# IannLiu/ReactRanker

Measured on AMD Instinct MI355X. Metric: queries/sec (lists scored+loss) ListMLE, higher is better.
Workload: dtype f32; 1 GPU; ListMLE 100k queries x 64 candidates (BASELINE.json configs[2]), 64-query steps, D-MPNN depth=3 hidden=300; preset=mle64, phase=train step: fwd + loss + bwd + grad all-reduce + Adam/NoamLR, candidates_per_query=64, pad_width_K=4, step_pool=6, parallelism=dp1

## Files before the change

### reactranker_amd/csrc/linear_common.h

```cpp
#pragma once
#include "rr_common.h"

namespace {

constexpr int BM = 64;
constexpr int BK = 16;
constexpr int THREADS = 256;

enum : int {
  F_A1_VEC = 1, F_A2_VEC = 2, F_SUB_VEC = 4, F_MASK_VEC = 8, F_W1_VEC = 16, F_W2_VEC = 32, F_EPI_VEC = 64, F_PRE_VEC = 128
};

__host__ __device__ constexpr int r16(int k) { return (k + 15) & ~15; }

struct LinearParams {
  rr_linear_args a;
  int w_k1_off;
  int t1, t2;
  int flags;
  uint32_t drop_thr;
  float keep_scale;
  int persist;
};

__device__ __forceinline__ f32x4 ld4(const float* p) { return *reinterpret_cast<const f32x4*>(p); }
typedef const __attribute__((address_space(1))) f32x4* rr_gptr4;
typedef const __attribute__((address_space(1))) int32_t* rr_gptri;
__device__ __forceinline__ f32x4 ldg4(const float* p) { return *(rr_gptr4)(p); }
__device__ __forceinline__ int32_t ldgi(const int32_t* p) { return *(rr_gptri)(p); }
typedef const __attribute__((address_space(1))) uint8_t* rr_gptrb;
__device__ __forceinline__ uint32_t ldgb(const uint8_t* p) { return *(rr_gptrb)(p); }
__host__ __device__ constexpr int64_t mask_bits_row(int N) { return 40 * ((N + 303) / 304); }

__device__ __forceinline__ void rr_glds16(const float* gsrc, uint32_t lds_dst) {
  uint32_t keep;
  asm volatile("s_mov_b32 %0, m0\n\ts_mov_b32 m0, %2\n\ts_nop 0\n\tglobal_load_lds_dwordx4 %1, off\n\ts_mov_b32 m0, %0"
               : "=&s"(keep)
               : "v"(gsrc), "s"(lds_dst)
               : "memory");
}
__device__ __forceinline__ void rr_wait_vm0() { asm volatile("s_waitcnt vmcnt(0)" ::: "memory"); }
__device__ __forceinline__ uint32_t rr_lds_addr(const float* p) {
  return static_cast<uint32_t>(reinterpret_cast<uintptr_t>((const __attribute__((address_space(3))) float*)p));
}

__device__ __forceinline__ f32x4 load_chunk(const float* p, int k, int ks, bool vec) {
  f32x4 v = f32x4(0.f);
  if (p == nullptr || k >= ks) return v;
  if (vec) {
    v = ld4(p + k);
    if (k + 3 >= ks) {
      if (k + 1 >= ks) v.y = 0.f;
      if (k + 2 >= ks) v.z = 0.f;
      v.w = 0.f;
    }
  } else {
    v.x = p[k];
    if (k + 1 < ks) v.y = p[k + 1];
    if (k + 2 < ks) v.z = p[k + 2];
    if (k + 3 < ks) v.w = p[k + 3];
  }
  return v;
}

__device__ __forceinline__ f32x4 apply_mask(f32x4 v, f32x4 mk, float scale) {
  v.x = mk.x > 0.f ? v.x * scale : 0.f;
  v.y = mk.y > 0.f ? v.y * scale : 0.f;
  v.z = mk.z > 0.f ? v.z * scale : 0.f;
  v.w = mk.w > 0.f ? v.w * scale : 0.f;
  return v;
}

#ifdef RR_TRACE
__device__ unsigned long long* rr_trace_buf = nullptr;
#define RR_STAMP(slot)                                                                                   \
  do {                                                                                                   \
    if (rr_trace_buf && threadIdx.x == 0 && blockIdx.y == 0) {                                           \
      rr_trace_buf[static_cast<size_t>(blockIdx.x) * 8 + (slot)] = __builtin_amdgcn_s_memrealtime();     \
      if ((slot) == 1) rr_trace_buf[static_cast<size_t>(blockIdx.x) * 8 + 5] = __builtin_amdgcn_s_memtime(); \
      if ((slot) == 2) rr_trace_buf[static_cast<size_t>(blockIdx.x) * 8 + 6] = __builtin_amdgcn_s_memtime(); \
    }                                                                                                    \
  } while (0)
inline int rr_trace_set_unit(unsigned long long* buf) {
  return hipMemcpyToSymbol(HIP_SYMBOL(rr_trace_buf), &buf, sizeof(buf)) == hipSuccess ? 0 : 1;
}
#else
#define RR_STAMP(slot)
#endif

__device__ __attribute__((aligned(16))) const float rr_zero_chunk[4] = {0.f, 0.f, 0.f, 0.f};
constexpr int RR_ZERO_ROW = 1024;
__device__ __attribute__((aligned(16))) const float rr_zero_row[RR_ZERO_ROW] = {0.f};

typedef __bf16 bf16x8 __attribute__((ext_vector_type(8)));
typedef uint32_t u32x4 __attribute__((ext_vector_type(4)));

constexpr int SK = 32;

__host__ __device__ constexpr int r32(int k) { return (k + 31) & ~31; }

__device__ __forceinline__ uint32_t cvt_pk_bf16(float lo, float hi) {
  uint32_t r;
  asm("v_cvt_pk_bf16_f32 %0, %1, %2" : "=v"(r) : "v"(lo), "v"(hi));
  return r;
}
__device__ __forceinline__ void split_pair(float x, float y, uint32_t& p0, uint32_t& p1, uint32_t& p2) {
  p0 = cvt_pk_bf16(x, y);
  float rx = x - __uint_as_float(p0 << 16), ry = y - __uint_as_float(p0 & 0xffff0000u);
  p1 = cvt_pk_bf16(rx, ry);
  rx -= __uint_as_float(p1 << 16);
  ry -= __uint_as_float(p1 & 0xffff0000u);
  p2 = cvt_pk_bf16(rx, ry);
}
__device__ __forceinline__ bf16x8 as_bf16x8(u32x4 v) { return __builtin_bit_cast(bf16x8, v); }
typedef _Float16 f16x8 __attribute__((ext_vector_type(8)));
typedef _Float16 f16x2 __attribute__((ext_vector_type(2)));
typedef float f32x2 __attribute__((ext_vector_type(2)));
__device__ __forceinline__ f16x8 as_f16x8(u32x4 v) { return __builtin_bit_cast(f16x8, v); }
__host__ __device__ __forceinline__ int rr_f16_exp(float bound) {
  uint32_t u;
  __builtin_memcpy(&u, &bound, 4);
  int e = static_cast<int>((u >> 23) & 0xffu) - 127;
  return e < -110 ? -110 : (e > 110 ? 110 : e);
}
__device__ __forceinline__ float rr_amax4(float m, f32x4 v) {
  return fmaxf(fmaxf(m, fmaxf(fabsf(v.x), fabsf(v.y))), fmaxf(fabsf(v.z), fabsf(v.w)));
}
__device__ __forceinline__ void rr_amax_commit_wave(float m, unsigned int* lds_word) {
#pragma unroll
  for (int o = 32; o > 0; o >>= 1) m = fmaxf(m, __shfl_xor(m, o));
  if ((threadIdx.x & 63) == 0 && m > 0.f) atomicMax(lds_word, __float_as_uint(m));
}
__device__ __forceinline__ float rr_pow2(int e) { return __uint_as_float(static_cast<uint32_t>(127 + e) << 23); }
__device__ __forceinline__ void split_pair_h(float x, float y, float S, uint32_t& p0, uint32_t& p1) {
  const f32x2 v = {x * S, y * S};
  const f16x2 h = __builtin_convertvector(v, f16x2);
  p0 = __builtin_bit_cast(uint32_t, h);
  const f32x2 r = v - __builtin_convertvector(h, f32x2);
  p1 = __builtin_bit_cast(uint32_t, __builtin_convertvector(r, f16x2));
}

inline bool vec_ok(const float* p, int64_t ld) { return p && rr_aligned16(p) && (ld % 4 == 0); }

inline LinearParams linear_params(const rr_linear_args& a) {
  LinearParams P;
  P.a = a;
  P.w_k1_off = a.w_packed ? r16(a.k1) : a.k1;
  P.t1 = (a.k1 + BK - 1) / BK;
  P.t2 = (a.k2 + BK - 1) / BK;
  P.flags = 0;
  P.persist = 0;
  if (a.k1 > 0 && vec_ok(a.a1, a.lda1)) P.flags |= F_A1_VEC;
  if (a.k2 > 0 && vec_ok(a.a2, a.lda2)) P.flags |= F_A2_VEC;
  if (a.a1_sub && vec_ok(a.a1_sub, a.lda1_sub)) P.flags |= F_SUB_VEC;
  if (a.a_mask && vec_ok(a.a_mask, a.ld_mask)) P.flags |= F_MASK_VEC;
  if (vec_ok(a.w, a.ldw)) {
    P.flags |= F_W1_VEC;
    if (a.k1 % 4 == 0) P.flags |= F_W2_VEC;
  }
  if (a.w_packed) P.flags |= F_W1_VEC | F_W2_VEC;
  if (a.N % 4 == 0 && vec_ok(a.c, a.ldc) && (!a.bias || rr_aligned16(a.bias)) &&
      (!a.residual || vec_ok(a.residual, a.ldr)))
    P.flags |= F_EPI_VEC;
  if (a.c_pre && vec_ok(a.c_pre, a.ld_pre)) P.flags |= F_PRE_VEC;
  P.drop_thr = rr_drop_threshold(a.drop_p);
  P.keep_scale = 1.0f / (1.0f - a.drop_p);
  return P;
}
}

extern "C" __attribute__((visibility("hidden"))) int rr_linear_split_launch(const rr_linear_args* args, int two_f16, rr_stream_t stream);
#ifdef RR_TRACE
extern "C" __attribute__((visibility("hidden"))) int rr_trace_set_linear_split(unsigned long long* buf);
extern "C" __attribute__((visibility("hidden"))) int rr_trace_set_wgrad(unsigned long long* buf);
#endif
```

### reactranker_amd/csrc/linear_split.hip

```cpp
#include "linear_common.h"
#include <atomic>

namespace {

#ifndef RR_EPI_MODE
#define RR_EPI_MODE 1
#endif

__host__ __device__ constexpr bool split_lean(int k1, int k2) { return k1 + SK <= RR_ZERO_ROW && k2 + SK <= RR_ZERO_ROW; }
__host__ __device__ constexpr bool split_can_persist(int NTP, int NT, int MODE, int WAVES, int EPI) {
  return MODE == 0 && WAVES == 12 && NT == NTP && EPI == 0;
}

template <int NTP, int NT, int MODE, int WAVES, int EPI = 0, bool F16 = false>
__global__ void __launch_bounds__(64 * WAVES, WAVES == 8 ? 4 : 3) linear_split_kernel(const LinearParams P) {
  constexpr int BN = 16 * NT;
  constexpr int TERMS = F16 ? 2 : 3;
  constexpr int PANEL = NT * TERMS * 1024;
  constexpr int SRC_PANEL = NTP * TERMS * 1024;
  constexpr int S_THREADS = 64 * WAVES;
  extern __shared__ __attribute__((aligned(16))) unsigned char smem[];
  constexpr bool RS_EPI = WAVES == 12;
  constexpr int RS = 77, REGION = 8 * RS * 16;
  constexpr int CS_OFF = RS_EPI ? (WAVES * REGION > 2 * PANEL ? WAVES * REGION : 2 * PANEL) : 0;
  constexpr int BIAS_OFF = RS_EPI ? CS_OFF + WAVES * BN * 4 : 2 * PANEL;
  float* const bias_s = reinterpret_cast<float*>(smem + BIAS_OFF);
  constexpr int PF_OFF = BIAS_OFF + BN * 4;
  constexpr bool PAIR = NTP == 2 * NT;
  const unsigned int bx = PAIR ? (((blockIdx.x >> 4) << 3) + (blockIdx.x & 7u)) : blockIdx.x;
  const unsigned int by = PAIR ? ((blockIdx.x >> 3) & 1u) : blockIdx.y;
  if (PAIR && static_cast<int64_t>(bx) * (16 * WAVES) >= P.a.M) return;
  const int t0 = by * NT;
  const int nth = NTP - t0 < NT ? NTP - t0 : NT;
  const bool full = nth == NT;
  const int n0 = t0 * 16;

  const rr_linear_args& a = P.a;
  const int tid = threadIdx.x, lane = tid & 63, wave = tid >> 6;
  const int fr = lane & 15, fkq = lane >> 4;
  float xs = 1.f, ixs = 1.f, iws = 1.f;
  if (F16) {
    float b1 = (a.a1_amax ? rr_amax_read(a.a1_amax) : 0.f) + (a.a1_sub_amax ? rr_amax_read(a.a1_sub_amax) : 0.f);
    if (MODE == 2 || MODE == 3) b1 *= fabsf(a.mask_scale);
    const float b2 = a.a2_amax ? rr_amax_read(a.a2_amax) : 0.f;
    const float bound = fmaxf(b1, b2);
    const int e = rr_f16_exp(bound);
    xs = bound < 2.5e33f ? rr_pow2(14 - e) : __builtin_nanf("");
    ixs = rr_pow2(e - 14);
    iws = 1.0f / a.w[static_cast<int64_t>(P.t1 + P.t2) * (SRC_PANEL / 4)];
  }
  RR_STAMP(0);
#ifdef RR_TRACE
  if (rr_trace_buf && threadIdx.x == 0 && by == 0) {
    unsigned hw, xcc;
    asm volatile("s_getreg_b32 %0, hwreg(HW_REG_HW_ID)" : "=s"(hw));
    asm volatile("s_getreg_b32 %0, hwreg(HW_REG_XCC_ID)" : "=s"(xcc));
    rr_trace_buf[static_cast<size_t>(bx) * 8 + 4] = (static_cast<unsigned long long>(xcc) << 32) | hw;
  }
#endif
#ifdef RR_SPLIT_STAGGER
  if (WAVES == 12 && gridDim.x > 256 && blockIdx.x < 256) {
    const int ph = (blockIdx.x >> 3) & 3;
    for (int i = 0; i < ph * RR_SPLIT_STAGGER; ++i) __builtin_amdgcn_s_sleep(127);
  }
#endif
  constexpr bool CAN_PERSIST = split_can_persist(NTP, NT, MODE, WAVES, EPI);
  const bool persist = CAN_PERSIST && P.persist != 0;
  unsigned int* const amx = reinterpret_cast<unsigned int*>(smem + PF_OFF + (CAN_PERSIST ? WAVES * 2048 : 0));
  if (F16 && tid == 0) { amx[0] = 0u; amx[1] = 0u; }
  int64_t g_cur = static_cast<int64_t>(bx) * WAVES;
  int64_t g_end = g_cur + WAVES;
  if (persist) {
    const int64_t units = (a.M + 63) / 64, G = gridDim.x;
    const int64_t base = units / G, rem = units % G, p = blockIdx.x;
    g_cur = 4 * (p * base + (p < rem ? p : rem));
    g_end = g_cur + 4 * (base + (p < rem ? 1 : 0));
  }
  int nw = g_end - g_cur < WAVES ? static_cast<int>(g_end - g_cur) : WAVES;
  int64_t m0 = g_cur * 16;
  int64_t m = m0 + wave * 16 + fr;
  bool row_ok = wave < nw && m < a.M;
  int64_t mc = row_ok ? m : a.M - 1;
  const float* const dummy = a.w;
  const float* rowp1 = nullptr;
  const float* rowp2 = nullptr;
  const float* subp = nullptr;
  const uint8_t* bitrow = nullptr;
  {
    const bool g1 = a.k1 > 0 && a.a1_idx != nullptr;
    const bool g2 = MODE == 1 && a.k1 > 0 && a.a1_sub != nullptr && a.a1_sub_idx != nullptr;
    const int32_t j1 = g1 ? ldgi(a.a1_idx + mc) : 0;
    const int32_t j2 = g2 ? ldgi(a.a1_sub_idx + mc) : 0;
    if (row_ok) {
      if (a.k1 > 0) {
        if (g1) {
          if (j1 >= 0) rowp1 = a.a1 + static_cast<int64_t>(j1) * a.lda1;
        } else {
          rowp1 = a.a1 + m * a.lda1;
        }
        if (MODE == 1 && a.a1_sub) {
          if (g2) {
            if (j2 >= 0) subp = a.a1_sub + static_cast<int64_t>(j2) * a.lda1_sub;
          } else {
            subp = a.a1_sub + m * a.lda1_sub;
          }
        }
        if (MODE == 2) subp = a.a_mask + m * a.ld_mask;
        if (MODE == 3) bitrow = a.a_mask_bits + m * mask_bits_row(a.k1);
      }
      if (a.k2 > 0) rowp2 = a.a2 + m * a.lda2;
    }
  }
  float dz_am = 0.f;
  float* dzrow = nullptr;
  if ((MODE == 2 || MODE == 3) && a.dz_out && row_ok && by == 0) dzrow = a.dz_out + m * a.ld_dz;

  const int uwave = __builtin_amdgcn_readfirstlane(wave);
  const float* const wlane = a.w + t0 * (TERMS * 256) + lane * 4;
  const uint32_t lds0 = rr_lds_addr(reinterpret_cast<const float*>(smem));

  f32x4 acc[NT];
#pragma unroll
  for (int i = 0; i < NT; ++i) acc[i] = f32x4(0.f);

  const int nk = P.t1 + P.t2;
  f32x4 ra[WAVES == 12 ? 2 : 1][2], rs[WAVES == 12 ? 2 : 1][2];
  uint32_t rb[2] = {0u, 0u};
  u32x4 x0, x1, x2;

#ifndef RR_SPLIT_NO_FASTX
  constexpr bool FASTX = (MODE == 0 || MODE == 1);
#else
  constexpr bool FASTX = false;
#endif
  static_assert(RR_ZERO_ROW % SK == 0 && RR_ZERO_ROW >= 2 * SK, "rr_zero_row must hold whole k-steps");
  constexpr bool LEAN_ONLY = FASTX && WAVES == 12 && EPI < 2;
  const bool fastx_ok = FASTX && (LEAN_ONLY || split_lean(a.k1, a.k2));
  const float* xb1 = (rowp1 != nullptr ? rowp1 : rr_zero_row) + fkq * 8;
  const float* xb2 = (rowp2 != nullptr ? rowp2 : rr_zero_row) + fkq * 8;
  const float* const sb1 = (subp != nullptr ? subp : rr_zero_row) + fkq * 8;
  const float* xb1n = xb1;
  const float* xb2n = xb2;
  bool has_next = false, wrapped = false;
  auto next_rows = [&](int64_t g, int nwn) {
    const int64_t mm = (g + wave) * 16 + fr;
    const bool ok = wave < nwn && mm < a.M;
    const int64_t mmc = ok ? mm : a.M - 1;
    const bool g1 = a.k1 > 0 && a.a1_idx != nullptr;
    const int32_t j1 = g1 ? ldgi(a.a1_idx + mmc) : 0;
    const float* r1 = nullptr;
    const float* r2 = nullptr;
    if (ok) {
      if (a.k1 > 0) {
        if (g1) {
          if (j1 >= 0) r1 = a.a1 + static_cast<int64_t>(j1) * a.lda1;
        } else {
          r1 = a.a1 + mm * a.lda1;
        }
      }
      if (a.k2 > 0) r2 = a.a2 + mm * a.lda2;
    }
    xb1n = (r1 != nullptr ? r1 : rr_zero_row) + fkq * 8;
    xb2n = (r2 != nullptr ? r2 : rr_zero_row) + fkq * 8;
  };
  auto interior = [&](int s) -> bool {
    if (!fastx_ok) return false;
    return s < P.t1 ? (s + 1) * SK <= a.k1 : (s - P.t1 + 1) * SK <= a.k2;
  };
  auto issue_x = [&](int s, int slot, bool nextblk = false) {
    if (FASTX && fastx_ok) {
      const bool s1 = s < P.t1;
      const int off = (s1 ? s : s - P.t1) * SK;
      const float* p = (s1 ? (nextblk ? xb1n : xb1) : (nextblk ? xb2n : xb2)) + off;
      const float* q = (MODE == 1 && s1) ? sb1 + off : rr_zero_row;
      if (interior(s)) {
        ra[slot][0] = ldg4(p);
        ra[slot][1] = ldg4(p + 4);
        if (MODE == 1) {
          rs[slot][0] = ldg4(q);
          rs[slot][1] = ldg4(q + 4);
        }
      } else {
        int fq = fkq;
        if (CAN_PERSIST) asm volatile("" : "+v"(fq));
        const int kl = off + fq * 8, ks = s1 ? a.k1 : a.k2;
        ra[slot][0] = ldg4(kl < ks ? p : rr_zero_row);
        ra[slot][1] = ldg4(kl + 4 < ks ? p + 4 : rr_zero_row);
        if (MODE == 1) {
          rs[slot][0] = ldg4(kl < ks ? q : rr_zero_row);
          rs[slot][1] = ldg4(kl + 4 < ks ? q + 4 : rr_zero_row);
        }
      }
      return;
    }
    const bool seg1 = s < P.t1;
    const int kl = (seg1 ? s : s - P.t1) * SK + fkq * 8;
    const float* p = seg1 ? rowp1 : rowp2;
    const int ks = seg1 ? a.k1 : a.k2;
    ra[slot][0] = ldg4((p != nullptr && kl < ks) ? p + kl : dummy);
    ra[slot][1] = ldg4((p != nullptr && kl + 4 < ks) ? p + kl + 4 : dummy);
    if (MODE == 1 || MODE == 2) {
      const bool oks = seg1 && subp != nullptr;
      rs[slot][0] = ldg4((oks && kl < ks) ? subp + kl : dummy);
      rs[slot][1] = ldg4((oks && kl + 4 < ks) ? subp + kl + 4 : dummy);
    }
    if (MODE == 3) {
      const int tc = 2 * s + (fkq >> 1);
      const int y = tc / 19;
      const uint8_t* q = bitrow + y * 40 + (fkq & 1) * 20 + (tc - 19 * y);
      rb[slot] = ldgb((seg1 && bitrow != nullptr && kl < ks) ? q : reinterpret_cast<const uint8_t*>(dummy));
    }
  };
  auto issue_w = [&](int s) {
    const float* src = wlane + static_cast<int64_t>(s) * (SRC_PANEL / 4);
    const uint32_t dst = lds0 + (s & 1) * PANEL;
#pragma unroll
    for (int b0 = 0; b0 < NT * TERMS; b0 += WAVES) {
      const int b = b0 + uwave;
      if (b < nth * TERMS) rr_glds16(src + b * 256, dst + b * 1024);
    }
  };
  auto split8 = [&](const f32x4& v0, const f32x4& v1) {
    uint32_t t0, t1, t2;
    if (F16) {
      split_pair_h(v0.x, v0.y, xs, t0, t1); x0.x = t0; x1.x = t1;
      split_pair_h(v0.z, v0.w, xs, t0, t1); x0.y = t0; x1.y = t1;
      split_pair_h(v1.x, v1.y, xs, t0, t1); x0.z = t0; x1.z = t1;
      split_pair_h(v1.z, v1.w, xs, t0, t1); x0.w = t0; x1.w = t1;
      return;
    }
    split_pair(v0.x, v0.y, t0, t1, t2); x0.x = t0; x1.x = t1; x2.x = t2;
    split_pair(v0.z, v0.w, t0, t1, t2); x0.y = t0; x1.y = t1; x2.y = t2;
    split_pair(v1.x, v1.y, t0, t1, t2); x0.z = t0; x1.z = t1; x2.z = t2;
    split_pair(v1.z, v1.w, t0, t1, t2); x0.w = t0; x1.w = t1; x2.w = t2;
  };
  auto fixup = [&](int s, int slot) {
    if (CAN_PERSIST && uwave >= nw) return;
    if (FASTX && fastx_ok) {
      f32x4 v0 = ra[slot][0], v1 = ra[slot][1];
      f32x4 u0 = f32x4(0.f), u1 = f32x4(0.f);
      if (MODE == 1) { u0 = rs[slot][0]; u1 = rs[slot][1]; }
      const bool s1 = s < P.t1;
      const int ks = s1 ? a.k1 : a.k2;
      if (!interior(s) && (ks & 3) != 0) {
        const int kl = (s1 ? s : s - P.t1) * SK + fkq * 8;
#pragma unroll
        for (int e = 0; e < 4; ++e) {
          v0[e] = kl + e < ks ? v0[e] : 0.f;
          v1[e] = kl + 4 + e < ks ? v1[e] : 0.f;
          if (MODE == 1) {
            u0[e] = kl + e < ks ? u0[e] : 0.f;
            u1[e] = kl + 4 + e < ks ? u1[e] : 0.f;
          }
        }
      }
      if (MODE == 1) {
        v0 = v0 - u0;
        v1 = v1 - u1;
      }
      split8(v0, v1);
      return;
    }
    const bool seg1 = s < P.t1;
    const int kl = (seg1 ? s : s - P.t1) * SK + fkq * 8;
    const float* p = seg1 ? rowp1 : rowp2;
    const int ks = seg1 ? a.k1 : a.k2;
    const bool ok = (p != nullptr);
    f32x4 v0, v1;
#pragma unroll
    for (int e = 0; e < 4; ++e) {
      v0[e] = (ok && kl + e < ks) ? ra[slot][0][e] : 0.f;
      v1[e] = (ok && kl + 4 + e < ks) ? ra[slot][1][e] : 0.f;
    }
    if (MODE == 1) {
      const bool oks = seg1 && (subp != nullptr);
#pragma unroll
      for (int e = 0; e < 4; ++e) {
        v0[e] -= (oks && kl + e < ks) ? rs[slot][0][e] : 0.f;
        v1[e] -= (oks && kl + 4 + e < ks) ? rs[slot][1][e] : 0.f;
      }
    }
    if (MODE == 2) {
      const bool oks = seg1 && (subp != nullptr);
#pragma unroll
      for (int e = 0; e < 4; ++e) {
        v0[e] = (oks && kl + e < ks && rs[slot][0][e] > 0.f) ? v0[e] * a.mask_scale : 0.f;
        v1[e] = (oks && kl + 4 + e < ks && rs[slot][1][e] > 0.f) ? v1[e] * a.mask_scale : 0.f;
      }
    }
    if (MODE == 3) {
      const bool oks = seg1 && (bitrow != nullptr);
      const uint32_t bits = rb[slot];
#pragma unroll
      for (int e = 0; e < 4; ++e) {
        v0[e] = (oks && kl + e < ks && ((bits >> e) & 1u)) ? v0[e] * a.mask_scale : 0.f;
        v1[e] = (oks && kl + 4 + e < ks && ((bits >> (4 + e)) & 1u)) ? v1[e] * a.mask_scale : 0.f;
      }
    }
    split8(v0, v1);
    if (MODE == 2 || MODE == 3) {
      if (dzrow != nullptr && seg1) {
        if (kl < ks) { *reinterpret_cast<f32x4*>(dzrow + kl) = v0; if (F16) dz_am = rr_amax4(dz_am, v0); }
        if (kl + 4 < ks) { *reinterpret_cast<f32x4*>(dzrow + kl + 4) = v1; if (F16) dz_am = rr_amax4(dz_am, v1); }
      }
    }
  };
  auto mfma_block = [&](int s) {
    if (CAN_PERSIST && uwave >= nw) return;
    const u32x4* Ws = reinterpret_cast<const u32x4*>(smem + (s & 1) * PANEL) + lane;
    if constexpr (F16) {
      const f16x8 h0 = as_f16x8(x0), h1 = as_f16x8(x1);
      u32x4 wa = Ws[0], wb = Ws[64];
      __builtin_amdgcn_sched_group_barrier(0x100, 2, 0);
#pragma unroll
      for (int j = 0; j < NT; ++j) {
        const f16x8 w0 = as_f16x8(wa), w1 = as_f16x8(wb);
        if (j + 1 < NT) {
          wa = Ws[((j + 1) * 2 + 0) * 64];
          wb = Ws[((j + 1) * 2 + 1) * 64];
        }
        f32x4 c = acc[j];
        if (j + 1 == NT && NT != NTP && !full) continue;
        c = __builtin_amdgcn_mfma_f32_16x16x32_f16(w1, h0, c, 0, 0, 0);
        c = __builtin_amdgcn_mfma_f32_16x16x32_f16(w0, h1, c, 0, 0, 0);
        c = __builtin_amdgcn_mfma_f32_16x16x32_f16(w0, h0, c, 0, 0, 0);
        acc[j] = c;
        if (j + 1 < NT) __builtin_amdgcn_sched_group_barrier(0x100, 2, 0);
        __builtin_amdgcn_sched_group_barrier(0x008, 3, 0);
      }
      return;
    }
    const bf16x8 b0 = as_bf16x8(x0), b1 = as_bf16x8(x1), b2 = as_bf16x8(x2);
    u32x4 wa = Ws[0], wb = Ws[64], wc = Ws[128];
    __builtin_amdgcn_sched_group_barrier(0x100, 3, 0);
#pragma unroll
    for (int j = 0; j < NT; ++j) {
      const bf16x8 w0 = as_bf16x8(wa), w1 = as_bf16x8(wb), w2 = as_bf16x8(wc);
      if (j + 1 < NT) {
        wa = Ws[((j + 1) * 3 + 0) * 64];
        wb = Ws[((j + 1) * 3 + 1) * 64];
        wc = Ws[((j + 1) * 3 + 2) * 64];
      }
      f32x4 c = acc[j];
      if (j + 1 == NT && NT != NTP && !full) continue;
      c = __builtin_amdgcn_mfma_f32_16x16x32_bf16(w2, b0, c, 0, 0, 0);
      c = __builtin_amdgcn_mfma_f32_16x16x32_bf16(w1, b1, c, 0, 0, 0);
      c = __builtin_amdgcn_mfma_f32_16x16x32_bf16(w0, b2, c, 0, 0, 0);
      c = __builtin_amdgcn_mfma_f32_16x16x32_bf16(w1, b0, c, 0, 0, 0);
      c = __builtin_amdgcn_mfma_f32_16x16x32_bf16(w0, b1, c, 0, 0, 0);
      c = __builtin_amdgcn_mfma_f32_16x16x32_bf16(w0, b0, c, 0, 0, 0);
      acc[j] = c;
      if (j + 1 < NT) __builtin_amdgcn_sched_group_barrier(0x100, 3, 0);
      __builtin_amdgcn_sched_group_barrier(0x008, 6, 0);
    }
  };
  constexpr int NX = MODE == 0 ? 2 : (MODE == 3 ? 3 : 4);
  constexpr bool DEEP = WAVES == 12;
#ifdef RR_SPLIT_NO_LATE
  const bool late = false;
#else
  const bool late = DEEP && uwave >= WAVES / 2;
#endif
  auto prefetch_next0 = [&]() {
    next_rows(g_cur + nw, g_end - (g_cur + nw) < WAVES ? static_cast<int>(g_end - (g_cur + nw)) : WAVES);
    const bool s1 = 0 < P.t1;
    const float* p = s1 ? xb1n : xb2n;
    const uint32_t dst = lds0 + PF_OFF + uwave * 2048;
    if (interior(0)) {
      rr_glds16(p, dst);
      rr_glds16(p + 4, dst + 1024);
    } else {
      int fq = fkq;
      asm volatile("" : "+v"(fq));
      const int kl = fq * 8, ks = s1 ? a.k1 : a.k2;
      rr_glds16(kl < ks ? p : rr_zero_row, dst);
      rr_glds16(kl + 4 < ks ? p + 4 : rr_zero_row, dst + 1024);
    }
  };
  auto step = [&](int s, int slot) {
    const bool more = s + 1 < nk, more2 = s + 2 < nk;
    const bool wrap = CAN_PERSIST && has_next;
    if (late && !(CAN_PERSIST && s == 0 && wrapped)) fixup(s, DEEP ? slot : 0);
    if (more) issue_w(s + 1);
    else if (wrap) issue_w(0);
    if (DEEP) {
      if (more2) issue_x(s + 2, slot);
      else if (wrap && more) prefetch_next0();
    } else {
      if (more) issue_x(s + 1, 0);
    }
    mfma_block(s);
    if (DEEP && (more2 || (wrap && more))) {
      if (NX == 2) asm volatile("s_waitcnt vmcnt(2)" ::: "memory");
      else if (NX == 3) asm volatile("s_waitcnt vmcnt(3)" ::: "memory");
      else asm volatile("s_waitcnt vmcnt(4)" ::: "memory");
    } else {
      rr_wait_vm0();
    }
    if (more && !late) fixup(s + 1, DEEP ? slot ^ 1 : 0);
    __syncthreads();
  };

  if (tid < BN / 4) {
    const int n = n0 + tid * 4;
    *reinterpret_cast<f32x4*>(bias_s + tid * 4) = ldg4((a.bias && n < a.N) ? a.bias + n : dummy);
  }
  issue_w(0);
  issue_x(0, 0);
  if (DEEP && nk > 1) issue_x(1, 1);
  rr_wait_vm0();
  if (!late) fixup(0, 0);
  __syncthreads();
  RR_STAMP(1);

  for (;;) {
  if (CAN_PERSIST) {
    has_next = persist && g_cur + nw < g_end;
  }
  for (int s = 0; s < nk; s += 2) {
    step(s, 0);
    if (s + 1 < nk) step(s + 1, 1);
  }
  RR_STAMP(2);

  if (F16) {
#pragma unroll
    for (int i = 0; i < NT; ++i) acc[i] = (acc[i] * ixs) * iws;
  }
  int lane_o = threadIdx.x;
#ifndef RR_PERSIST_HOIST
  if (CAN_PERSIST) asm volatile("" : "+v"(lane_o));
#endif
  const int tid = lane_o, lane = lane_o & 63, wave = lane_o >> 6;
  const int fr = lane & 15, fkq = lane >> 4;
  const int64_t m0 = g_cur * 16;
  const int64_t m = m0 + wave * 16 + fr;
  const bool row_ok = wave < nw && m < a.M;
  const int64_t mc = row_ok ? m : a.M - 1;
  const int nq = fkq * 4;
  float* crow = a.c + mc * a.ldc;
  const float* rrow = nullptr;
  if (a.residual) {
    const int64_t rr = a.residual_idx ? static_cast<int64_t>(a.residual_idx[mc]) : mc;
    if (rr >= 0) rrow = a.residual + rr * a.ldr;
  }
  const bool has_bias = a.bias != nullptr;
  const bool relu = a.act == RR_ACT_RELU;
  float c_am = 0.f;
  auto finish = [&](f32x4 v, int n) -> f32x4 {
    if (relu) {
#pragma unroll
      for (int e = 0; e < 4; ++e) v[e] = fmaxf(v[e], 0.f);
    }
    if (P.drop_thr != 0u) {
      const uint64_t base = static_cast<uint64_t>(m) * static_cast<uint64_t>(a.N) + static_cast<uint64_t>(n);
      const uint32_t w = rr_hash_group(a.drop_seed, base >> 2);
#pragma unroll
      for (int e = 0; e < 4; ++e) v[e] = rr_hash_lane(w, e) >= P.drop_thr ? v[e] * P.keep_scale : 0.f;
    }
    if (row_ok && n < a.N) {
      *reinterpret_cast<f32x4*>(crow + n) = v;
      if (F16) c_am = rr_amax4(c_am, v);
    }
    return v;
  };
  float* prow = a.c_pre ? a.c_pre + mc * a.ld_pre : nullptr;
  const bool mb_on = a.mask_bits_out != nullptr;
  uint32_t mb[5] = {0u, 0u, 0u, 0u, 0u};
  const bool cs_on = a.colsum_partial != nullptr;
  const float wrow = (cs_on && row_ok) ? a.colsum_w[mc] : 0.f;
  float* const cs_lds = reinterpret_cast<float*>(smem + CS_OFF);
  const bool plain_epi = !has_bias && a.residual == nullptr && !relu && P.drop_thr == 0u && prow == nullptr && !mb_on;
  bool done = false;
  if (RS_EPI && (EPI & 1) == 1 && (!cs_on || plain_epi)) {
    done = true;
    if (cs_on) {
#pragma unroll
      for (int tc = 0; tc < NT; ++tc) {
        f32x4 t = acc[tc] * wrow;
#pragma unroll
        for (int e = 0; e < 4; ++e) {
          float x = t[e];
          x += __int_as_float(__builtin_amdgcn_update_dpp(0, __float_as_int(x), 0x111, 0xf, 0xf, true));
          x += __int_as_float(__builtin_amdgcn_update_dpp(0, __float_as_int(x), 0x112, 0xf, 0xf, true));
          x += __int_as_float(__builtin_amdgcn_update_dpp(0, __float_as_int(x), 0x114, 0xf, 0xf, true));
          x += __int_as_float(__builtin_amdgcn_update_dpp(0, __float_as_int(x), 0x118, 0xf, 0xf, true));
          t[e] = x;
        }
        if (fr == 15) *reinterpret_cast<f32x4*>(cs_lds + wave * BN + tc * 16 + nq) = t;
      }
    }
    unsigned char* const region = smem + uwave * REGION;
    unsigned char* const bits_s = smem + CS_OFF + uwave * 640;
    if (mb_on) {
#pragma unroll
      for (int d = lane; d < 160; d += 64) reinterpret_cast<uint32_t*>(bits_s)[d] = 0u;
    }
    const int nqv = (a.N - n0) / 4 < 4 * NT ? (a.N - n0) / 4 : 4 * NT;
    const int64_t mw = m0 + uwave * 16;
    const bool res_on = a.residual != nullptr;
    constexpr int NI = (8 * 76 + 63) / 64;
#pragma unroll
    for (int pass = 0; pass < 2; ++pass) {
      if ((fr >> 3) == pass) {
#pragma unroll
        for (int tc = 0; tc < NT; ++tc)
          *reinterpret_cast<f32x4*>(region + (((fr & 7) * RS + tc * 4 + fkq) << 4)) = acc[tc];
      }
      constexpr int RG = 2;
#pragma unroll
      for (int i0 = 0; i0 < NI; i0 += RG) {
        asm volatile("" ::: "memory");
        f32x4 rres[RG];
#pragma unroll
        for (int u = 0; u < RG; ++u) {
          const int i = i0 + u;
          if (i < NI && res_on) {
            const int q = (64 * i) / 76, rem = (64 * i) % 76;
            const bool wrap = rem + lane >= 76;
            const int r = q + (wrap ? 1 : 0), c4 = rem + lane - (wrap ? 76 : 0);
            const int64_t mm = mw + pass * 8 + r;
            const bool ok = (64 * i + lane < 8 * 76) && c4 < nqv && mm < a.M;
            const int64_t mmc = ok ? mm : 0;
            const int64_t rr = a.residual_idx ? static_cast<int64_t>(ldgi(a.residual_idx + mmc)) : mmc;
            rres[u] = ldg4((ok && rr >= 0) ? a.residual + rr * a.ldr + n0 + 4 * c4 : rr_zero_chunk);
          }
        }
#pragma unroll
        for (int u = 0; u < RG; ++u) {
          const int i = i0 + u;
          if (i >= NI) continue;
          const int q = (64 * i) / 76, rem = (64 * i) % 76;
          const bool wrap = rem + lane >= 76;
          const int r = q + (wrap ? 1 : 0), c4 = rem + lane - (wrap ? 76 : 0);
          const int64_t mm = mw + pass * 8 + r;
          const bool ok = (64 * i + lane < 8 * 76) && c4 < nqv && mm < a.M;
          const int n = n0 + 4 * c4;
          f32x4 v = *reinterpret_cast<const f32x4*>(region + ((r * RS + c4) << 4));
          if (has_bias) v = v + *reinterpret_cast<const f32x4*>(bias_s + 4 * (c4 < 4 * NT ? c4 : 0));
          if (res_on) v = v + rres[u];
          if (prow != nullptr && ok) *reinterpret_cast<f32x4*>(a.c_pre + mm * a.ld_pre + n) = v;
          if (relu) {
#pragma unroll
            for (int e = 0; e < 4; ++e) v[e] = fmaxf(v[e], 0.f);
          }
          if (P.drop_thr != 0u) {
            const uint64_t base = static_cast<uint64_t>(mm) * static_cast<uint64_t>(a.N) + static_cast<uint64_t>(n);
            const uint32_t w = rr_hash_group(a.drop_seed, base >> 2);
#pragma unroll
            for (int e = 0; e < 4; ++e) v[e] = rr_hash_lane(w, e) >= P.drop_thr ? v[e] * P.keep_scale : 0.f;
          }
          if (ok) {
            *reinterpret_cast<f32x4*>(a.c + mm * a.ldc + n) = v;
            if (F16) c_am = rr_amax4(c_am, v);
          }
          if (mb_on) {
            uint32_t nib = (v.x > 0.f ? 1u : 0u) | (v.y > 0.f ? 2u : 0u) | (v.z > 0.f ? 4u : 0u) | (v.w > 0.f ? 8u : 0u);
            if (c4 >= nqv) nib = 0u;
            const uint32_t other = static_cast<uint32_t>(__builtin_amdgcn_ds_bpermute((lane ^ 1) << 2, static_cast<int>(nib)));
            const int j = c4 >> 1;
            if ((c4 & 1) == 0 && 64 * i + lane < 8 * 76 && c4 < 4 * NT)
              bits_s[(pass * 8 + r) * 40 + (j & 1) * 20 + (j >> 1)] = static_cast<uint8_t>(nib | (other << 4));
          }
        }
      }
    }
    if (mb_on) {
      const int64_t rowb = mask_bits_row(a.N);
#pragma unroll
      for (int d = lane; d < 160; d += 64) {
        const int r = d / 10, w = d - 10 * r;
        if (mw + r < a.M)
          *reinterpret_cast<uint32_t*>(a.mask_bits_out + (mw + r) * rowb + by * 40 + 4 * w) = reinterpret_cast<const uint32_t*>(bits_s)[d];
      }
    }
  }
  if (!done) {
    constexpr bool MAY_RES = !(RR_EPI_MODE == 1 && WAVES == 12 && (MODE == 0 || MODE == 1) && (EPI & 1) == 0);
    const bool res_ok = MAY_RES && rrow != nullptr;
    const float* rbase = res_ok ? rrow : dummy;
    constexpr int D = MAY_RES ? 4 : 0;
    f32x4 ring[D + 1];
    auto ldres = [&](int tc) {
      const int n = n0 + tc * 16 + nq;
      return ldg4(rbase + ((res_ok && n < a.N) ? n : 0));
    };
#pragma unroll
    for (int t = 0; t < D; ++t)
      if (t < NT) ring[t] = ldres(t);
#pragma unroll
    for (int tc = 0; tc < NT; ++tc) {
      const int n = n0 + tc * 16 + nq;
      const f32x4 b = *reinterpret_cast<const f32x4*>(bias_s + tc * 16 + nq);
      f32x4 v = acc[tc];
      const f32x4 vb = v + b;
#pragma unroll
      for (int e = 0; e < 4; ++e) v[e] = has_bias ? vb[e] : v[e];
      if (MAY_RES) {
        const f32x4 vr = v + ring[tc % (D + 1)];
#pragma unroll
        for (int e = 0; e < 4; ++e) v[e] = res_ok ? vr[e] : v[e];
        if (tc + D < NT) ring[(tc + D) % (D + 1)] = ldres(tc + D);
      }
      if (prow != nullptr && row_ok && n < a.N) *reinterpret_cast<f32x4*>(prow + n) = v;
      const f32x4 stored = finish(v, n);
      if (mb_on) {
        const uint32_t nib = (stored.x > 0.f ? 1u : 0u) | (stored.y > 0.f ? 2u : 0u) | (stored.z > 0.f ? 4u : 0u) | (stored.w > 0.f ? 8u : 0u);
        const uint32_t other = static_cast<uint32_t>(__builtin_amdgcn_ds_bpermute((lane ^ 16) << 2, static_cast<int>(nib)));
        if (NT == 19) {
          mb[tc >> 2] |= (nib | (other << 4)) << (8 * (tc & 3));
        } else if (row_ok && (fkq & 1) == 0 && (full || tc + 1 < NT)) {
          const int tg = t0 + tc;
          a.mask_bits_out[m * mask_bits_row(a.N) + (tg / 19) * 40 + (fkq >> 1) * 20 + (tg % 19)] =
              static_cast<uint8_t>(nib | (other << 4));
        }
      }
      if (cs_on) {
        f32x4 t = stored * wrow;
#pragma unroll
        for (int e = 0; e < 4; ++e) {
          float x = t[e];
          x += __int_as_float(__builtin_amdgcn_update_dpp(0, __float_as_int(x), 0x111, 0xf, 0xf, true));
          x += __int_as_float(__builtin_amdgcn_update_dpp(0, __float_as_int(x), 0x112, 0xf, 0xf, true));
          x += __int_as_float(__builtin_amdgcn_update_dpp(0, __float_as_int(x), 0x114, 0xf, 0xf, true));
          x += __int_as_float(__builtin_amdgcn_update_dpp(0, __float_as_int(x), 0x118, 0xf, 0xf, true));
          t[e] = x;
        }
        if (fr == 15) *reinterpret_cast<f32x4*>(cs_lds + wave * BN + tc * 16 + nq) = t;
      }
    }
  }
  if (!done && NT == 19 && mb_on && row_ok && (fkq & 1) == 0) {
    uint32_t* d = reinterpret_cast<uint32_t*>(a.mask_bits_out + m * mask_bits_row(a.N) + by * 40 + (fkq >> 1) * 20);
#pragma unroll
    for (int i = 0; i < 5; ++i) d[i] = mb[i];
  }
  if (F16 && a.c_amax_out != nullptr) rr_amax_commit_wave(c_am, amx);
  if (F16 && (MODE == 2 || MODE == 3) && a.dz_amax_out != nullptr && by == 0) {
    rr_amax_commit_wave(dz_am, amx + 1);
    dz_am = 0.f;
  }
  if (cs_on) {
    __syncthreads();
    static_assert(WAVES % 4 == 0 && (WAVES / 4) * (BN / 4) <= S_THREADS, "colsum slices");
    if (tid < (WAVES / 4) * (BN / 4)) {
      const int h = tid / (BN / 4);
      const int q = tid - h * (BN / 4);
      const int n = n0 + q * 4;
      const float* base = cs_lds + h * 4 * BN + q * 4;
      const f32x4 s01 = ld4(base) + ld4(base + BN);
      const f32x4 s23 = ld4(base + 2 * BN) + ld4(base + 3 * BN);
      if (n < a.N && h * 4 < nw && m0 + h * 64 < a.M)
        *reinterpret_cast<f32x4*>(a.colsum_partial + (g_cur / 4 + h) * a.ld_partial + n) = s01 + s23;
    }
  }
  if (!(CAN_PERSIST && has_next)) break;
  if (cs_on) __syncthreads();
  wrapped = true;
  g_cur += nw;
  nw = g_end - g_cur < WAVES ? static_cast<int>(g_end - g_cur) : WAVES;
  next_rows(g_cur, nw);
  xb1 = xb1n;
  xb2 = xb2n;
  if (nk > 1) issue_x(1, 1);
  {
    const unsigned char* pf = smem + PF_OFF + uwave * 2048 + lane * 16;
    ra[0][0] = *reinterpret_cast<const f32x4*>(pf);
    ra[0][1] = *reinterpret_cast<const f32x4*>(pf + 1024);
  }
  fixup(0, 0);
#pragma unroll
  for (int i = 0; i < NT; ++i) acc[i] = f32x4(0.f);
  }
  if (F16 && (a.c_amax_out != nullptr || a.dz_amax_out != nullptr)) {
    __syncthreads();
    if (threadIdx.x == 0) {
      const unsigned int vc = amx[0], vd = amx[1];
      if (a.c_amax_out != nullptr) rr_amax_put(a.c_amax_out, __uint_as_float(vc));
      if (a.dz_amax_out != nullptr) rr_amax_put(a.dz_amax_out, __uint_as_float(vd));
    }
  }
#ifdef RR_TRACE
  asm volatile("s_waitcnt vmcnt(0)" ::: "memory");
  RR_STAMP(3);
#endif
}

template <int NTP, int NT, int MODE, int WAVES, int EPI, bool F16>
int launch_split_epi(const LinearParams& P, hipStream_t s) {
  constexpr int panel2 = 2 * NT * (F16 ? 2 : 3) * 1024, bn4 = 16 * NT * 4;
  constexpr bool can_persist = split_can_persist(NTP, NT, MODE, WAVES, EPI);
  constexpr int smem = (WAVES == 12 ? ((12 * 8 * 77 * 16 > panel2 ? 12 * 8 * 77 * 16 : panel2) + 13 * bn4) : panel2 + bn4) +
                       (can_persist ? WAVES * 2048 : 0) + 16;
  static std::atomic<uint64_t> configured{0};
  int dev = 0;
  if (hipGetDevice(&dev) != hipSuccess) return RR_ERR_LAUNCH;
  if (dev < 0 || dev >= 64 || !((configured.load(std::memory_order_acquire) >> dev) & 1u)) {
    if (hipFuncSetAttribute(reinterpret_cast<const void*>(&linear_split_kernel<NTP, NT, MODE, WAVES, EPI, F16>),
                            hipFuncAttributeMaxDynamicSharedMemorySize, smem) != hipSuccess)
      return RR_ERR_LAUNCH;
    if (dev >= 0 && dev < 64) configured.fetch_or(uint64_t(1) << dev, std::memory_order_release);
  }
  const int64_t nblk = (P.a.M + 16 * WAVES - 1) / (16 * WAVES);
  if (can_persist) {
    static int n_cu[64] = {0};
    int cus = (dev >= 0 && dev < 64) ? n_cu[dev] : 0;
    if (cus == 0) {
      if (hipDeviceGetAttribute(&cus, hipDeviceAttributeMultiprocessorCount, dev) != hipSuccess || cus < 1) cus = 1 << 30;
      if (dev >= 0 && dev < 64) n_cu[dev] = cus;
    }
    const int nk = P.t1 + P.t2;
    if (nblk > cus && nk >= 2 && nk % 2 == 0 && split_lean(P.a.k1, P.a.k2) && !getenv("RR_NO_PERSIST")) {
      LinearParams Q = P;
      Q.persist = 1;
      const dim3 grid(static_cast<unsigned>(cus), 1);
      linear_split_kernel<NTP, NT, MODE, WAVES, EPI, F16><<<grid, 64 * WAVES, smem, s>>>(Q);
      return rr_launch_status();
    }
  }
  const dim3 grid = NTP == 2 * NT ? dim3(static_cast<unsigned>((nblk + 7) / 8 * 16), 1)
                                  : dim3(static_cast<unsigned>(nblk), static_cast<unsigned>((NTP + NT - 1) / NT));
  linear_split_kernel<NTP, NT, MODE, WAVES, EPI, F16><<<grid, 64 * WAVES, smem, s>>>(P);
  return rr_launch_status();
}
template <int NTP, int NT, int MODE, int WAVES, bool F16>
int launch_split_one(const LinearParams& P, hipStream_t s) {
  if (WAVES == 12 && (MODE == 0 || MODE == 1)) {
    const bool rs = RR_EPI_MODE == 2 || (RR_EPI_MODE == 1 && P.a.residual != nullptr);
    const bool lean = split_lean(P.a.k1, P.a.k2);
    constexpr int E1 = (WAVES == 12 && (MODE == 0 || MODE == 1)) ? 1 : 0, G = (WAVES == 12 && (MODE == 0 || MODE == 1)) ? 2 : 0;
    if (!lean) return rs ? launch_split_epi<NTP, NT, MODE, WAVES, G + E1, F16>(P, s) : launch_split_epi<NTP, NT, MODE, WAVES, G, F16>(P, s);
    if (rs) return launch_split_epi<NTP, NT, MODE, WAVES, E1, F16>(P, s);
  }
  return launch_split_epi<NTP, NT, MODE, WAVES, 0, F16>(P, s);
}
template <int NTP, int NT, int WAVES, bool F16>
int launch_split(const LinearParams& P, hipStream_t s) {
  if (P.a.a_mask_bits) return launch_split_one<NTP, NT, 3, WAVES, F16>(P, s);
  if (P.a.a_mask) return launch_split_one<NTP, NT, 2, WAVES, F16>(P, s);
  if (P.a.a1_sub) return launch_split_one<NTP, NT, 1, WAVES, F16>(P, s);
  return launch_split_one<NTP, NT, 0, WAVES, F16>(P, s);
}
template <bool F16>
int launch_split_geometry(const LinearParams& P, hipStream_t s) {
  const rr_linear_args& a = P.a;
  if (a.N <= 64) return launch_split<4, 4, 8, F16>(P, s);
  if (a.N <= 160) return launch_split<10, 10, 8, F16>(P, s);
  if (a.N <= 304 && a.M <= 8192) return launch_split<19, 5, 8, F16>(P, s);
  if (a.N <= 304) return launch_split<19, 19, 12, F16>(P, s);
  return launch_split<38, 19, 12, F16>(P, s);
}
}

extern "C" {

#ifdef RR_TRACE
int rr_trace_set_linear_split(unsigned long long* buf) { return rr_trace_set_unit(buf); }
#endif

int rr_linear_split_launch(const rr_linear_args* args, int two_f16, rr_stream_t stream) {
  LinearParams P = linear_params(*args);
  P.t1 = r32(P.a.k1) / SK;
  P.t2 = r32(P.a.k2) / SK;
  hipStream_t s = static_cast<hipStream_t>(stream);
  return two_f16 ? launch_split_geometry<true>(P, s) : launch_split_geometry<false>(P, s);
}

}
```

Baseline: 12800 queries/s.

## Balance tail wave of split linear kernel across all CUs

For non-persistent 12-wave split GEMM variants, the launch now counts 64-row units and, when the last wave of blocks would only partly fill the CUs, spreads the leftover units evenly over one block per CU instead of leaving a few full blocks. Blocks beyond the full-size region handle fewer units and idle waves skip the fixup, MFMA and epilogue work. This targets tail-wave imbalance (wave quantization) in the row-blocked linear kernels. In exchange the kernel gets extra index arithmetic and an asm barrier on the block descriptor, and partially filled blocks still hold the full 12-wave shared-memory footprint.

```diff
diff --git a/reactranker_amd/csrc/linear_common.h b/reactranker_amd/csrc/linear_common.h
--- a/reactranker_amd/csrc/linear_common.h
+++ b/reactranker_amd/csrc/linear_common.h
@@ -21,6 +21,7 @@
   uint32_t drop_thr;
   float keep_scale;
   int persist;
+  int bal_full, bal_base, bal_rem;
 };
 
 __device__ __forceinline__ f32x4 ld4(const float* p) { return *reinterpret_cast<const f32x4*>(p); }
@@ -150,6 +151,7 @@
   P.t2 = (a.k2 + BK - 1) / BK;
   P.flags = 0;
   P.persist = 0;
+  P.bal_full = P.bal_base = P.bal_rem = 0;
   if (a.k1 > 0 && vec_ok(a.a1, a.lda1)) P.flags |= F_A1_VEC;
   if (a.k2 > 0 && vec_ok(a.a2, a.lda2)) P.flags |= F_A2_VEC;
   if (a.a1_sub && vec_ok(a.a1_sub, a.lda1_sub)) P.flags |= F_SUB_VEC;
diff --git a/reactranker_amd/csrc/linear_split.hip b/reactranker_amd/csrc/linear_split.hip
--- a/reactranker_amd/csrc/linear_split.hip
+++ b/reactranker_amd/csrc/linear_split.hip
@@ -10,6 +10,10 @@
 __host__ __device__ constexpr bool split_lean(int k1, int k2) { return k1 + SK <= RR_ZERO_ROW && k2 + SK <= RR_ZERO_ROW; }
 __host__ __device__ constexpr bool split_can_persist(int NTP, int NT, int MODE, int WAVES, int EPI) {
   return MODE == 0 && WAVES == 12 && NT == NTP && EPI == 0;
+}
+
+__host__ __device__ constexpr bool split_balanced(int NTP, int NT, int MODE, int WAVES, int EPI, bool F16) {
+  return WAVES == 12 && NT == NTP && EPI < 2 && !F16 && !split_can_persist(NTP, NT, MODE, WAVES, EPI);
 }
 
 template <int NTP, int NT, int MODE, int WAVES, int EPI = 0, bool F16 = false>
@@ -28,7 +32,9 @@
   constexpr int PF_OFF = BIAS_OFF + BN * 4;
   constexpr bool PAIR = NTP == 2 * NT;
   const unsigned int bx = PAIR ? (((blockIdx.x >> 4) << 3) + (blockIdx.x & 7u)) : blockIdx.x;
-  const unsigned int by = PAIR ? ((blockIdx.x >> 3) & 1u) : blockIdx.y;
+  constexpr bool BALANCED = split_balanced(NTP, NT, MODE, WAVES, EPI, F16);
+  constexpr bool SHORT = BALANCED || split_can_persist(NTP, NT, MODE, WAVES, EPI);
+  const unsigned int by = PAIR ? ((blockIdx.x >> 3) & 1u) : (BALANCED ? 0u : blockIdx.y);
   if (PAIR && static_cast<int64_t>(bx) * (16 * WAVES) >= P.a.M) return;
   const int t0 = by * NT;
   const int nth = NTP - t0 < NT ? NTP - t0 : NT;
@@ -75,6 +81,18 @@
     const int64_t base = units / G, rem = units % G, p = blockIdx.x;
     g_cur = 4 * (p * base + (p < rem ? p : rem));
     g_end = g_cur + 4 * (base + (p < rem ? 1 : 0));
+  }
+  int blk = 0;
+  if (BALANCED) {
+    int u0 = static_cast<int>(blockIdx.x) * (WAVES / 4), nu = WAVES / 4;
+    if ((P.bal_base | P.bal_rem) != 0 && static_cast<int>(blockIdx.x) >= P.bal_full) {
+      const int q = static_cast<int>(blockIdx.x) - P.bal_full;
+      u0 = P.bal_full * (WAVES / 4) + q * P.bal_base + (q < P.bal_rem ? q : P.bal_rem);
+      nu = P.bal_base + (q < P.bal_rem ? 1 : 0);
+    }
+    blk = (u0 << 2) | nu;
+    g_cur = 4 * static_cast<int64_t>(u0);
+    g_end = g_cur + 4 * nu;
   }
   int nw = g_end - g_cur < WAVES ? static_cast<int>(g_end - g_cur) : WAVES;
   int64_t m0 = g_cur * 16;
@@ -235,7 +253,7 @@
     split_pair(v1.z, v1.w, t0, t1, t2); x0.w = t0; x1.w = t1; x2.w = t2;
   };
   auto fixup = [&](int s, int slot) {
-    if (CAN_PERSIST && uwave >= nw) return;
+    if (SHORT && uwave >= nw) return;
     if (FASTX && fastx_ok) {
       f32x4 v0 = ra[slot][0], v1 = ra[slot][1];
       f32x4 u0 = f32x4(0.f), u1 = f32x4(0.f);
@@ -306,7 +324,7 @@
     }
   };
   auto mfma_block = [&](int s) {
-    if (CAN_PERSIST && uwave >= nw) return;
+    if (SHORT && uwave >= nw) return;
     const u32x4* Ws = reinterpret_cast<const u32x4*>(smem + (s & 1) * PANEL) + lane;
     if constexpr (F16) {
       const f16x8 h0 = as_f16x8(x0), h1 = as_f16x8(x1);
@@ -433,9 +451,13 @@
 #endif
   const int tid = lane_o, lane = lane_o & 63, wave = lane_o >> 6;
   const int fr = lane & 15, fkq = lane >> 4;
-  const int64_t m0 = g_cur * 16;
+  int blk_o = blk;
+  if (BALANCED) asm volatile("" : "+s"(blk_o));
+  const int64_t gb = BALANCED ? 4 * static_cast<int64_t>(blk_o >> 2) : g_cur;
+  const int nwb = BALANCED ? 4 * (blk_o & 3) : nw;
+  const int64_t m0 = gb * 16;
   const int64_t m = m0 + wave * 16 + fr;
-  const bool row_ok = wave < nw && m < a.M;
+  const bool row_ok = wave < nwb && m < a.M;
   const int64_t mc = row_ok ? m : a.M - 1;
   const int nq = fkq * 4;
   float* crow = a.c + mc * a.ldc;
@@ -471,8 +493,9 @@
   const float wrow = (cs_on && row_ok) ? a.colsum_w[mc] : 0.f;
   float* const cs_lds = reinterpret_cast<float*>(smem + CS_OFF);
   const bool plain_epi = !has_bias && a.residual == nullptr && !relu && P.drop_thr == 0u && prow == nullptr && !mb_on;
-  bool done = false;
-  if (RS_EPI && (EPI & 1) == 1 && (!cs_on || plain_epi)) {
+  const bool idle = BALANCED && uwave >= nwb;
+  bool done = idle;
+  if (!idle && RS_EPI && (EPI & 1) == 1 && (!cs_on || plain_epi)) {
     done = true;
     if (cs_on) {
 #pragma unroll
@@ -650,8 +673,8 @@
       const float* base = cs_lds + h * 4 * BN + q * 4;
       const f32x4 s01 = ld4(base) + ld4(base + BN);
       const f32x4 s23 = ld4(base + 2 * BN) + ld4(base + 3 * BN);
-      if (n < a.N && h * 4 < nw && m0 + h * 64 < a.M)
-        *reinterpret_cast<f32x4*>(a.colsum_partial + (g_cur / 4 + h) * a.ld_partial + n) = s01 + s23;
+      if (n < a.N && h * 4 < nwb && m0 + h * 64 < a.M)
+        *reinterpret_cast<f32x4*>(a.colsum_partial + (gb / 4 + h) * a.ld_partial + n) = s01 + s23;
     }
   }
   if (!(CAN_PERSIST && has_next)) break;
@@ -686,6 +709,15 @@
 #endif
 }
 
+inline int split_cus(int dev) {
+  static std::atomic<int> n_cu[64];
+  int cus = (dev >= 0 && dev < 64) ? n_cu[dev].load(std::memory_order_relaxed) : 0;
+  if (cus == 0) {
+    if (hipDeviceGetAttribute(&cus, hipDeviceAttributeMultiprocessorCount, dev) != hipSuccess || cus < 1) cus = 1 << 30;
+    if (dev >= 0 && dev < 64) n_cu[dev].store(cus, std::memory_order_relaxed);
+  }
+  return cus;
+}
 template <int NTP, int NT, int MODE, int WAVES, int EPI, bool F16>
 int launch_split_epi(const LinearParams& P, hipStream_t s) {
   constexpr int panel2 = 2 * NT * (F16 ? 2 : 3) * 1024, bn4 = 16 * NT * 4;
@@ -702,18 +734,28 @@
     if (dev >= 0 && dev < 64) configured.fetch_or(uint64_t(1) << dev, std::memory_order_release);
   }
   const int64_t nblk = (P.a.M + 16 * WAVES - 1) / (16 * WAVES);
+  if (split_balanced(NTP, NT, MODE, WAVES, EPI, F16) && nblk >= (int64_t(1) << 27)) return RR_ERR_UNSUPPORTED;
+  const int cus = split_cus(dev);
   if (can_persist) {
-    static int n_cu[64] = {0};
-    int cus = (dev >= 0 && dev < 64) ? n_cu[dev] : 0;
-    if (cus == 0) {
-      if (hipDeviceGetAttribute(&cus, hipDeviceAttributeMultiprocessorCount, dev) != hipSuccess || cus < 1) cus = 1 << 30;
-      if (dev >= 0 && dev < 64) n_cu[dev] = cus;
-    }
     const int nk = P.t1 + P.t2;
     if (nblk > cus && nk >= 2 && nk % 2 == 0 && split_lean(P.a.k1, P.a.k2) && !getenv("RR_NO_PERSIST")) {
       LinearParams Q = P;
       Q.persist = 1;
       const dim3 grid(static_cast<unsigned>(cus), 1);
+      linear_split_kernel<NTP, NT, MODE, WAVES, EPI, F16><<<grid, 64 * WAVES, smem, s>>>(Q);
+      return rr_launch_status();
+    }
+  }
+  if (split_balanced(NTP, NT, MODE, WAVES, EPI, F16) && nblk > cus && !getenv("RR_NO_BALANCED_TAIL") &&
+      !(MODE >= 2 && getenv("RR_NO_BALANCED_TAIL_DX"))) {
+    const int64_t units = (P.a.M + 63) / 64;
+    const int64_t full = units / (3 * static_cast<int64_t>(cus)) * cus, tail = units - 3 * full;
+    if (tail > 0 && tail <= 2 * static_cast<int64_t>(cus)) {
+      LinearParams Q = P;
+      Q.bal_full = static_cast<int>(full);
+      Q.bal_base = static_cast<int>(tail / cus);
+      Q.bal_rem = static_cast<int>(tail % cus);
+      const dim3 grid(static_cast<unsigned>(full + (Q.bal_base > 0 ? cus : Q.bal_rem)), 1);
       linear_split_kernel<NTP, NT, MODE, WAVES, EPI, F16><<<grid, 64 * WAVES, smem, s>>>(Q);
       return rr_launch_status();
     }
```

Result: faster. 12970 queries/s, median of 6 (+1.3%).
